# fengpeng-yue/speech-to-speech-translation

Hardware: AMD Instinct MI355X
Metric: mel-frames/sec (fwd+bwd+opt) on Fisher-shaped fbank80->mel80 (higher is better)
Workload: dtype bf16; 1 GPU; s2st_transformer base 12enc/6dec d512 nfps4 + aux ASR/ST(1x64) + CTC, recipe dropouts, max-tokens=20000 Fisher-shaped batches, update-freq 1; parallelism=dp1

## Files before the change

speech-to-speech-translation_amd/csrc/gemm_bf16.hip:

```cpp
#include "gemm_bf16_tile.h"
#include "gemm_bf16_launch.h"

namespace {

template <int BM, int BN, bool AKM, bool BKM, bool VEC>
__global__ __launch_bounds__(256) void gemm_bf16_kernel(GemmArgs g) {
  constexpr int WM = BM / 2, WN = BN / 2, TM = WM / 16, TN = WN / 16;
  typedef Stage<AKM, BM, VEC> LA;
  typedef Stage<BKM, BN, VEC> LB;
  constexpr int A_BYTES = LA::BYTES, B_BYTES = LB::BYTES, STAGE = A_BYTES + B_BYTES;
  __shared__ __attribute__((aligned(16))) unsigned char smem[2 * STAGE];

  const int tid = threadIdx.x;
  const int wave = tid >> 6, lane = tid & 63;
  const int wm = wave >> 1, wn = wave & 1;

  const int nwg = gridDim.x;
  int id = blockIdx.x;
  {
    const int x = id & 7, q = nwg >> 3, r = nwg & 7;
    id = (x < r ? x * (q + 1) : r * (q + 1) + (x - r) * q) + (id >> 3);
  }
  const int tile_m = id / g.tiles_n, tile_n = id - tile_m * g.tiles_n;
  const int m0 = tile_m * BM, n0 = tile_n * BN;
// ... 663 lines not shown
  const int z = blockIdx.y, zq = z / zdiv, zr = z - zq * zdiv;
  const float* sp = slab + ((long)z * splitk * M + m) * N + n;
  float* cp = C.p + zq * C.zo + zr * C.zi + split_off(C.sp, m) + n;
  const long sstride = (long)M * N;
  if ((N & 3) == 0 && ((uintptr_t)cp & 15) == 0) {
    float4 a = accumulate ? *reinterpret_cast<const float4*>(cp) : make_float4(0.f, 0.f, 0.f, 0.f);
    for (int sb = 0; sb < splitk; sb += 8) {
      float4 v[8];
#pragma unroll
      for (int j = 0; j < 8; ++j) v[j] = *reinterpret_cast<const float4*>(sp + (long)min(sb + j, splitk - 1) * sstride);
#pragma unroll
      for (int j = 0; j < 8; ++j)
        if (sb + j < splitk) { a.x += v[j].x; a.y += v[j].y; a.z += v[j].z; a.w += v[j].w; }
    }
    *reinterpret_cast<float4*>(cp) = a;
  } else {
    for (int r = 0; r < 4 && n + r < N; ++r) {
      float a = accumulate ? cp[r] : 0.f;
      for (int s = 0; s < splitk; ++s) a += sp[s * sstride + r];
      cp[r] = a;
    }
  }
}

template <int BM, int BN, bool VEC>
int launch_staged(const GemmArgs& g, dim3 grid, hipStream_t st) {
  return with_layouts(g, [&](auto a, auto b) {
    constexpr bool AKM = decltype(a)::value, BKM = decltype(b)::value;
    return launch_configured<GEMM_STAGED, BM, BN, AKM, BKM, VEC>(gemm_bf16_kernel<BM, BN, AKM, BKM, VEC>, 0, grid, 256, st, g);
  });
}

constexpr bool kExperimental =
#ifdef S2ST_EXPERIMENTAL
    true;
#else
    false;
#endif
static_assert(GEMM_BK == BK, "the plan prices the kernels' K-step");

enum SwitchScope { SW_MEMBER, SW_GROUP, SW_SINGLE };
GemmSwitches gemm_switches(SwitchScope scope) {
  static const int dma = s2st_env_int("S2ST_GEMM_DMA", 1), target = s2st_env_int("S2ST_SPLITK_TARGET", 128),
                   wgs = s2st_env_int("S2ST_GEMM_PERSIST_WGS", 0);
  GemmSwitches sw;
  sw.dma = dma;
  sw.splitk_target = target;
  sw.persist_wgs = wgs;
  sw.persist = s2st_env_int("S2ST_GEMM_PERSIST", sw.persist);
  if (!kExperimental && sw.persist > 1) sw.persist = 1;
  if (scope == SW_MEMBER) return sw;
  sw.w4 = s2st_env_int("S2ST_GEMM_W4", sw.w4);
  sw.fast_epi = s2st_env_int("S2ST_GEMM_FAST_EPI", 1) != 0;
  sw.streamk = kExperimental ? s2st_env_int("S2ST_GEMM_STREAMK", 1) : 0;
  if (sw.streamk > 0) sw.streamk_min_steps = s2st_env_int("S2ST_STREAMK_MIN_STEPS", sw.streamk_min_steps);
  if (scope == SW_GROUP) {
    sw.group_tile = s2st_env_int("S2ST_GROUP_TILE", 0);
    sw.group_oneshot = s2st_env_int("S2ST_GROUP_ONESHOT", 1) != 0;
    return sw;
  }
  sw.p4 = s2st_env_int("S2ST_GEMM_P4", sw.p4);
  if (const char* force = s2st_env_str("S2ST_GEMM_TILE")) {
    sw.tile_set = true;
    if (sscanf(force, "%dx%d", &sw.tile_bm, &sw.tile_bn) != 2) sw.tile_bm = sw.tile_bn = 64;
  }
  return sw;
}

GemmChip gemm_chip(const GemmSwitches& sw, int ncu = 0, int slots160 = 0) {
  return GemmChip{ncu > 0 ? ncu : num_cus(sw), slots160 > 0 ? slots160 : s2st_gemm_bf16_w4_slots160(), kExperimental};
}

GemmGroup group_of(const GemmArgs* list, const GemmPlan& p) {
  GemmGroup grp{};
  grp.n = p.n;
  grp.total = p.total;
  for (int i = 0; i < p.n; ++i) {
    GemmArgs& g = grp.g[i] = list[i];
    if (g.zdiv <= 0) g.zdiv = 1;
    g.avec = g.bvec = p.vec;
    g.cvec = p.cvec_of[i];
    g.splitk = 1;
    g.slab = nullptr;
    g.kchunk = ((g.K + BK - 1) / BK) * BK;
    g.tiles_n = (g.N + p.bn - 1) / p.bn;
    grp.tile0[i + 1] = p.tile0[i + 1];
  }
  return grp;
}

}

void s2st_gemm_streamk_bind(hipStream_t st, float* scratch, long floats) {
  if (floats < S2ST_STREAMK_SCRATCH_FLOATS) scratch = nullptr;
  for (int i = 0; i < g_sk_n; ++i)
    if (g_sk[i].st == st) { g_sk[i].p = scratch; return; }
  if (g_sk_n < 4) g_sk[g_sk_n++] = SkScratch{st, scratch};
}
void s2st_gemm_streamk_unbind_all() { g_sk_n = 0; }

bool s2st_gemm_group_ok(const GemmArgs& g) {
  return group_member_ok(g, gemm_switches(SW_MEMBER));
}

int s2st_gemm_bf16_group(const GemmArgs* list, int n, hipStream_t st) {
  if (n <= 0) return 0;
  const GemmSwitches sw = gemm_switches(SW_GROUP);
  const GemmPlan p = plan_group(list, n, sw, gemm_chip(sw), sk_scratch(st) != nullptr);
  if (p.error) return p.error;
  GemmGroup grp = group_of(list, p);
  grp.xcd_global = 1;
  int rc = S2ST_ERR_ARG;
  switch (p.form) {
    case GEMM_GROUP_RING: rc = launch_group_ring(grp, st); break;
    case GEMM_GROUP_W4: rc = s2st_gemm_bf16_w4_group(grp, st); break;
#ifdef S2ST_EXPERIMENTAL
    case GEMM_GROUP_PERSISTENT: rc = launch_persistent<128, 128>(grp, p.sk, p.grid_x, st); break;
    case GEMM_GROUP_PERSISTENT_256: rc = launch_persistent<256, 128>(grp, p.sk, p.grid_x, st); break;
#endif
    default: break;
  }
  return rc == 0 && hipGetLastError() == hipSuccess ? 0 : S2ST_ERR_LAUNCH;
}

int s2st_gemm_bf16_preload(hipStream_t st) {
  dim3 grid(1, 1, 1);
  int rc = 0;
  for (int lay = 0; lay < 4; ++lay) {
    const GemmArgs g = empty_problem(lay);
    rc |= launch_staged<128, 128, true>(g, grid, st);
    rc |= launch_staged<128, 64, true>(g, grid, st);
    rc |= launch_staged<64, 64, true>(g, grid, st);
    rc |= launch_staged<64, 64, false>(g, grid, st);
    rc |= launch_ring<128, 128>(g, grid, st);
    rc |= launch_ring<128, 64>(g, grid, st);
    if (g.A.kmajor) rc |= launch_ring<160, 64>(g, grid, st);
    rc |= launch_ring<64, 64>(g, grid, st);
    GemmGroup grp{};
    grp.n = 1;
    grp.g[0] = g;
#ifdef S2ST_EXPERIMENTAL
    rc |= launch_persistent<128, 128>(grp, false, 1, st);
    rc |= launch_persistent<128, 64>(grp, false, 1, st);
    rc |= launch_persistent<256, 128>(grp, false, 1, st);
    rc |= launch_ring<256, 128>(g, grid, st);
#endif
    rc |= launch_group_ring(grp, st);
  }
  rc |= s2st_gemm_bf16_w4_preload(st);
  rc |= s2st_gemm_bf16_p4_preload(st);
  return rc || hipGetLastError() != hipSuccess ? -1 : 0;
}

int s2st_gemm_bf16(GemmArgs g, hipStream_t st, int* tile_out) {
  const GemmSwitches sw = gemm_switches(SW_SINGLE);
  const GemmPlan p = plan_single(g, sw, gemm_chip(sw), sk_scratch(st) != nullptr);
  if (p.error) return p.error;
  g.avec = g.bvec = p.vec;
  g.cvec = p.cvec;
  g.splitk = p.splitk;
  g.kchunk = p.kchunk;
  g.tiles_n = p.tiles_n;
  g.slab = p.use_slab ? g.ws : nullptr;
  if (tile_out) *tile_out = p.bm * 1000 + p.bn;
  const dim3 grid(p.grid_x, p.grid_y, 1);
  const bool wide = p.bn == 128;
  int rc = S2ST_ERR_ARG;
  switch (p.form) {
    case GEMM_STAGED:
      rc = !p.vec ? launch_staged<64, 64, false>(g, grid, st) : p.bm == 64 ? launch_staged<64, 64, true>(g, grid, st)
           : wide ? launch_staged<128, 128, true>(g, grid, st) : launch_staged<128, 64, true>(g, grid, st);
      break;
    case GEMM_RING:
      rc = p.bm == 160 ? launch_ring<160, 64>(g, grid, st) : p.bm == 64 ? launch_ring<64, 64>(g, grid, st)
           : wide ? launch_ring<128, 128>(g, grid, st) : launch_ring<128, 64>(g, grid, st);
      break;
    case GEMM_W4: rc = s2st_gemm_bf16_w4(g, p.bm, p.bn, grid, st); break;
    case GEMM_P4: rc = s2st_gemm_bf16_p4(g, grid, st); break;
#ifdef S2ST_EXPERIMENTAL
    case GEMM_RING_256x128: rc = launch_ring<256, 128>(g, grid, st); break;
    case GEMM_PERSISTENT:
      rc = wide ? launch_persistent<128, 128>(group_of(&g, p), p.sk, p.grid_x, st)
                : launch_persistent<128, 64>(group_of(&g, p), p.sk, p.grid_x, st);
      break;
#endif
    default: break;
  }
  if (rc) return rc;
  if (p.use_slab) {
    const long nthr = (long)g.M * ((g.N + 3) / 4);
    const double by = 4.0 * g.M * g.N * g.batch * (g.splitk + 1 + (g.ep.accumulate ? 1 : 0));
    s2st_launch("splitk_reduce_kernel", by, 0.0, splitk_reduce_kernel, dim3((unsigned)((nthr + 255) / 256), g.batch),
                dim3(256), 0, st, (const float*)g.slab, g.C, g.M, g.N, g.splitk, g.zdiv, g.ep.accumulate);
  }
  return hipGetLastError() == hipSuccess ? 0 : -1;
}

int s2st_gemm_bf16_plan(const GemmArgs* list, int n, int ncu, int slots160, bool sk_bound, s2st_gemm_plan_info* out) {
  const GemmSwitches sw = gemm_switches(n ? SW_GROUP : SW_SINGLE);
  const GemmChip chip = gemm_chip(sw, ncu, slots160);
  GemmPlan p;
  if (list[0].A.dtype != S2ST_BF16 || list[0].B.dtype != S2ST_BF16 || list[0].precise) p.error = S2ST_ERR_ARG;
  else if (n == 0) p = plan_single(list[0], sw, chip, sk_bound);
  else {
    for (int i = 0; i < n && !p.error; ++i)
      if (!group_member_ok(list[i], sw)) p.error = S2ST_ERR_SHAPE;
    if (!p.error) p = plan_group(list, n, sw, chip, sk_bound);
  }
  *out = s2st_gemm_plan_info{p.error};
  if (p.error) return 0;
  *out = s2st_gemm_plan_info{0, (int)p.form, p.bm, p.bn, p.splitk, p.kchunk, p.tiles_n, p.use_slab, p.vec, p.cvec, p.grid_x, p.grid_y,
                             p.sk, p.n, p.total};
// ... 218 lines not shown
```

speech-to-speech-translation_amd/csrc/gemm_bf16_plan.h:

```cpp
#pragma once
#include <stdint.h>
#include <stdio.h>
#include "s2st_hip.h"

typedef s2st_gemm_operand GemmOperand;
typedef s2st_gemm_args GemmArgs;

constexpr int GEMM_BK = 64;
#define S2ST_GROUP_MAX 8
#define S2ST_STREAMK_MAX_WGS 512
#define S2ST_STREAMK_SCRATCH_FLOATS (1024 + (long)S2ST_STREAMK_MAX_WGS * 128 * 128)

struct GemmSwitches {
  int dma = 1;
  bool tile_set = false;
  int tile_bm = 64, tile_bn = 64;
  int w4 = -1;
  int p4 = -1;
  int persist = 1;
  int persist_wgs = 0;
  int streamk = 1;
  int streamk_min_steps = 8;
  bool fast_epi = true;
  int splitk_target = 128;
  int group_tile = 0;
  bool group_oneshot = true;
};

struct GemmChip { int ncu; int slots160; bool experimental; };

enum GemmForm {
  GEMM_STAGED, GEMM_RING, GEMM_W4, GEMM_P4, GEMM_PERSISTENT, GEMM_RING_256x128,
  GEMM_GROUP_RING, GEMM_GROUP_W4, GEMM_GROUP_PERSISTENT, GEMM_GROUP_PERSISTENT_256
};

struct GemmPlan {
  int error = 0;
  GemmForm form = GEMM_STAGED;
  int bm = 0, bn = 0, splitk = 1, kchunk = 0, tiles_n = 0, vec = 0, cvec = 0, grid_x = 0, grid_y = 1;
  bool use_slab = false;
  bool akm = false, bkm = false;
  bool sk = false;
  int n = 0, total = 0, tile0[S2ST_GROUP_MAX + 1] = {0}, cvec_of[S2ST_GROUP_MAX] = {0};
};

constexpr int ring_ns(int bm) { return bm == 256 ? 3 : 4; }
constexpr int ring_nw(int bm) { return bm == 64 ? 4 : 8; }
constexpr bool ring_il(int bm) { return bm != 256; }
constexpr int W4_NS = 2;

inline void gemm_tag(char* buf, size_t cap, GemmForm f, int bm, int bn, bool akm, bool bkm, bool last) {
  const char *a = akm ? "true" : "false", *b = bkm ? "true" : "false", *l = last ? "true" : "false";
  switch (f) {
    case GEMM_STAGED: snprintf(buf, cap, "gemm_bf16_kernel<%d, %d, %s, %s, %s>", bm, bn, a, b, l); break;
    case GEMM_RING: case GEMM_RING_256x128: case GEMM_GROUP_RING:
      snprintf(buf, cap, "gemm_bf16_dma%s_kernel<%d, %d, %s, %s, %d, %d, %s>", f == GEMM_GROUP_RING ? "_group" : "", bm, bn, a, b,
               ring_ns(bm), ring_nw(bm), ring_il(bm) ? "true" : "false");
      break;
    case GEMM_W4: case GEMM_GROUP_W4:
      snprintf(buf, cap, "gemm_bf16_w4%s_kernel<%d, %d, %s, %s, %d>", f == GEMM_GROUP_W4 ? "_group" : "", bm, bn, a, b, W4_NS);
      break;
    case GEMM_P4: snprintf(buf, cap, "gemm_bf16_p4_kernel<256, 256>"); break;
    default:
      snprintf(buf, cap, "gemm_bf16_dma_persistent_kernel<%d, %d, %s, %s, %d, %d, %s>", bm, bn, a, b, ring_ns(bm), ring_nw(bm), l);
  }
}

inline long gemm_tiles(const GemmArgs& g, int bm, int bn) { return (long)((g.M + bm - 1) / bm) * ((g.N + bn - 1) / bn) * g.batch; }

inline bool vec_ok(const GemmOperand& o) {
  return ((uintptr_t)o.p % 16 == 0) && (o.sp.ld % 8 == 0) && (o.sp.bs % 8 == 0) && (o.zo % 8 == 0) && (o.zi % 8 == 0);
}

inline bool dma_layout_ok(const GemmArgs& g) { return (g.A.kmajor || g.A.sp.per <= 0) && (g.B.kmajor || g.B.sp.per <= 0); }

inline bool prep_flags(const GemmArgs& g, int* cvec) {
  *cvec = ((!g.C.p || (uintptr_t)g.C.p % 16 == 0) && (!g.C.h || (uintptr_t)g.C.h % 8 == 0) &&
           g.C.sp.ld % 4 == 0 && g.C.sp.bs % 4 == 0 && g.C.zo % 4 == 0 && g.C.zi % 4 == 0 &&
           (!g.ep.resid || (uintptr_t)g.ep.resid % 16 == 0) && (!g.ep.bias || ((uintptr_t)g.ep.bias % 16 == 0 && g.ep.bias_zo % 4 == 0)))
              ? 1 : 0;
  return vec_ok(g.A) && vec_ok(g.B);
}

inline int mark_fast_epilogue(const GemmArgs& g, int cvec, bool unsplit, const GemmSwitches& sw) {
  cvec &= 1;
  if (!sw.fast_epi) return cvec;
  const bool drop = g.ep.drop_p > 0.f, res = g.ep.resid != nullptr, accu = g.ep.accumulate != 0;
  const bool combo = !accu || (!drop && !res && !g.C.h);
  const bool h16 = !g.C.h || ((uintptr_t)g.C.h % 16 == 0 && g.C.sp.ld % 8 == 0 && g.C.sp.bs % 8 == 0 && g.C.zo % 8 == 0 &&
                              g.C.zi % 8 == 0 && g.N % 8 == 0);
  if (cvec && g.N >= 4 && g.N % 4 == 0 && g.M >= 1 && unsplit && !g.ep.mask_y && !g.ep.colsum && !g.ep.colsum_part &&
      (g.ep.act != 2 || (!drop && !accu)) && combo && h16 && (g.C.p || g.C.h) && (!accu || g.C.p))
    cvec |= 2;
  if (cvec && g.ep.mask_y && g.C.h && !g.C.p && h16 && g.N >= 8 && g.M >= 1 && unsplit && !g.ep.bias &&
      g.ep.act == 0 && !drop && !res && !accu && (uintptr_t)g.ep.mask_y % 16 == 0)
    cvec |= 8;
  return cvec;
}

inline bool tile160_ok(const GemmArgs& g) { return g.A.kmajor && g.A.sp.per <= 0 && g.batch == 1; }

inline int w4_pick(const GemmArgs& g, const GemmSwitches& sw, const GemmChip& chip, int* bm) {
  *bm = 128;
  if (sw.w4 == 0 || g.M < 128) return 0;
  const long t128 = gemm_tiles(g, 128, 128), t64 = gemm_tiles(g, 128, 64);
  if (sw.w4 < 0 && t128 < chip.ncu) return 0;
  const long s128 = 2L * chip.ncu, s64 = 3L * chip.ncu;
  const double e128 = (double)t128 / (double)(((t128 + s128 - 1) / s128) * s128);
  const double e64 = (double)t64 / (double)(((t64 + s64 - 1) / s64) * s64);
  if (tile160_ok(g) && g.N > 64) {
    const long t160 = gemm_tiles(g, 160, 128);
    const long s160 = (long)chip.slots160 * chip.ncu;
    if (t160 <= s160 && t128 > s128 && t64 > s64) { *bm = 160; return 128; }
  }
  if (g.N > 64 && g.K >= 1024 && t128 >= 4 * s128) return 128;
  return (g.N > 64 && e128 >= e64) ? 128 : 64;
}

inline bool p4_can(const GemmArgs& g) {
  return g.A.kmajor && g.B.kmajor && g.batch == 1 && g.A.sp.per <= 0 && g.B.sp.per <= 0 && !g.ep.mask_y &&
         !g.ep.colsum && !g.ep.colsum_part;
}
inline bool p4_pick(const GemmArgs& g, const GemmSwitches& sw, const GemmChip& chip) {
  if (sw.p4 >= 1) return true;
  if (g.M < 512 || g.N < 512 || g.K < 8 * GEMM_BK) return false;
  const long ncu = chip.ncu;
  const long rounds = (gemm_tiles(g, 256, 256) + ncu - 1) / ncu;
  const double t_p4 = (double)rounds * (2.0 * ((g.K + GEMM_BK - 1) / GEMM_BK) + 7.0);
  const double t_ring = 2.0 * g.M * (double)g.N * g.K / 650e6;
  return t_p4 < 0.80 * t_ring;
}

inline bool streamk_pays(long total, long steps, const GemmSwitches& sw, const GemmChip& chip) {
  const int G = chip.ncu & ~7;
// ... 160 lines not shown
```

speech-to-speech-translation_amd/csrc/gemm_bf16_tile.h:

```cpp
#pragma once
#include <cstdio>
#include <cstdlib>

#include "s2st_ops.h"
#include "s2st_prof.h"

namespace {

typedef unsigned short bf16_t;
constexpr int BK = 64;

template <int ROWS>
__device__ __forceinline__ int kperm(int kr) {
  if (ROWS >= 128) return (kr & 3) | (((kr >> 3) & 1) << 2);
  return ((kr >> 1) & 1) | (((kr >> 3) & 1) << 1);
}

__device__ __forceinline__ uint4 mask_tail(uint4 v, int nvalid) {
  unsigned w[4] = {v.x, v.y, v.z, v.w};
#pragma unroll
  for (int i = 0; i < 4; ++i) {
    int e = nvalid - 2 * i;
    w[i] = e >= 2 ? w[i] : (e == 1 ? (w[i] & 0xffffu) : 0u);
  }
// ... 74 lines not shown
      if (KM) {
        const int row = f >> 3, ch = f & 7;
        o = row * 128 + ((ch ^ (row & 7)) << 4);
      } else {
        const int kr = f / RC, ch = f % RC;
        o = kr * PITCH + (((((ch >> 1) ^ kperm<ROWS>(kr)) << 1) | (ch & 1)) << 4);
      }
      *reinterpret_cast<uint4*>(img + o) = r[i];
    }
  }

  struct Raw { bf16x8 v; s16x4 lo, hi; };
  __device__ static __forceinline__ Raw raw(const unsigned char* img, int rt, int s, int lane) {
    Raw r;
    if (KM) {
      r.v = frag(img, rt, s, lane);
    } else {
      const int g = lane >> 4, q = (lane >> 2) & 3, p = lane & 3;
      const int kr = 32 * s + 8 * g + q;
      const unsigned char* a = img + kr * PITCH + ((((rt >> 4) ^ kperm<ROWS>(kr))) << 5) + 8 * p;
      r.lo = lds_read_tr16_raw(a);
      r.hi = lds_read_tr16_raw(a + 4 * PITCH);
    }
    return r;
  }
  __device__ static __forceinline__ bf16x8 done(Raw& r) {
    if (KM) return r.v;
    lds_raw_fence(r.lo);
    lds_raw_fence(r.hi);
    bf16x8 fr;
    fr[0] = r.lo[0]; fr[1] = r.lo[1]; fr[2] = r.lo[2]; fr[3] = r.lo[3];
    fr[4] = r.hi[0]; fr[5] = r.hi[1]; fr[6] = r.hi[2]; fr[7] = r.hi[3];
    return fr;
  }

  __device__ static __forceinline__ bf16x8 frag(const unsigned char* img, int rt, int s, int lane) {
    if (KM) {
      const int row = rt + (lane & 15), ch = 4 * s + (lane >> 4);
      return *reinterpret_cast<const bf16x8*>(img + row * 128 + ((ch ^ (row & 7)) << 4));
    } else {
      const int g = lane >> 4, q = (lane >> 2) & 3, p = lane & 3;
      const int kr = 32 * s + 8 * g + q;
      const unsigned char* a = img + kr * PITCH + ((((rt >> 4) ^ kperm<ROWS>(kr))) << 5) + 8 * p;
      s16x4 lo = lds_read_tr16(a);
      s16x4 hi = lds_read_tr16(a + 4 * PITCH);
      bf16x8 fr;
      fr[0] = lo[0]; fr[1] = lo[1]; fr[2] = lo[2]; fr[3] = lo[3];
      fr[4] = hi[0]; fr[5] = hi[1]; fr[6] = hi[2]; fr[7] = hi[3];
      return fr;
    }
  }
};

template <int BM, int BN, int WGN, bool DROP, bool RESID, bool ACC, bool HASC, bool HASH, bool H16, bool GELU = false>
__device__ __forceinline__ void gemm_epilogue_fast(const GemmArgs& g, f32x4 (&acc)[BM / 32][BN / (16 * WGN)], int m0, int n0,
                                                   int wm, int wn, int lane, int zb, int zq, int zr,
                                                   const float4 (*pre)[BN / (16 * WGN)]) {
  constexpr int WM = BM / 2, WN = BN / WGN, TM = WM / 16, TN = WN / 16;
  const long czoff = zq * g.C.zo + zr * g.C.zi;
  float* cbase = g.C.p + czoff;
  bf16_t* hbase = g.C.h + czoff;
  const float* rbase = g.ep.resid + czoff;
  const int M = g.M, N = g.N;
  const float alpha = g.ep.alpha, lo = g.ep.act == 1 ? 0.f : -__builtin_inff();
  const float drop_p = g.ep.drop_p, inv_keep = DROP ? 1.f / (1.f - drop_p) : 1.f;
  const uint64_t seed = g.ep.seed;
  int ncol[TN];
  bool nok[TN];
  float4 b4[TN];
#pragma unroll
  for (int j = 0; j < TN; ++j) {
    const int n = n0 + wn * WN + j * 16 + (lane >> 4) * 4;
    nok[j] = n < N;
    ncol[j] = nok[j] ? n : N - 4;
    b4[j] = make_float4(0.f, 0.f, 0.f, 0.f);
  }
  if (g.ep.bias) {
    const float* bias = g.ep.bias + zq * g.ep.bias_zo;
#pragma unroll
    for (int j = 0; j < TN; ++j) b4[j] = *reinterpret_cast<const float4*>(bias + ncol[j]);
  }
  long roff[TM];
  int mrow[TM];
  bool mok[TM];
#pragma unroll
  for (int i = 0; i < TM; ++i) {
    const int m = m0 + wm * WM + i * 16 + (lane & 15);
    mok[i] = m < M;
    mrow[i] = mok[i] ? m : M - 1;
    roff[i] = split_off(g.C.sp, mrow[i]);
  }
  float4 r4[RESID ? TM : 1][RESID ? TN : 1], c4[ACC ? TM : 1][ACC ? TN : 1];
  if (RESID) {
#pragma unroll
    for (int i = 0; i < TM; ++i)
#pragma unroll
      for (int j = 0; j < TN; ++j)
        r4[RESID ? i : 0][RESID ? j : 0] = pre ? pre[i][j] : *reinterpret_cast<const float4*>(rbase + roff[i] + ncol[j]);
  }
  if (ACC) {
#pragma unroll
    for (int i = 0; i < TM; ++i)
#pragma unroll
      for (int j = 0; j < TN; ++j)
        c4[ACC ? i : 0][ACC ? j : 0] = pre ? pre[i][j] : *reinterpret_cast<const float4*>(cbase + roff[i] + ncol[j]);
  }
  uint2 hp[(HASH && H16) ? TM : 1][(HASH && H16) ? TN : 1];
#pragma unroll
  for (int i = 0; i < TM; ++i) {
#pragma unroll
    for (int j = 0; j < TN; ++j) {
      float v[4] = {fmaxf(alpha * acc[i][j][0] + b4[j].x, lo), fmaxf(alpha * acc[i][j][1] + b4[j].y, lo),
                    fmaxf(alpha * acc[i][j][2] + b4[j].z, lo), fmaxf(alpha * acc[i][j][3] + b4[j].w, lo)};
      if (GELU) {
#pragma unroll
        for (int r = 0; r < 4; ++r) v[r] = gelu_erf_fast(v[r]);
      }
      if (DROP) {
        const uint64_t e0 = ((uint64_t)zb * M + mrow[i]) * (uint64_t)N + ncol[j];
#pragma unroll
        for (int r = 0; r < 4; ++r) v[r] *= drop_scale(seed, e0 + r, drop_p, inv_keep);
      }
      if (RESID) {
        const float4 t = r4[RESID ? i : 0][RESID ? j : 0];
        v[0] += t.x; v[1] += t.y; v[2] += t.z; v[3] += t.w;
      }
      if (ACC) {
        const float4 t = c4[ACC ? i : 0][ACC ? j : 0];
        v[0] += t.x; v[1] += t.y; v[2] += t.z; v[3] += t.w;
      }
      if (mok[i] && nok[j]) {
        if (HASC) *reinterpret_cast<float4*>(cbase + roff[i] + ncol[j]) = make_float4(v[0], v[1], v[2], v[3]);
        if (HASH && !H16) *reinterpret_cast<uint2*>(hbase + roff[i] + ncol[j]) = pack_bf16x4(v[0], v[1], v[2], v[3]);
      }
      if (HASH && H16) hp[(HASH && H16) ? i : 0][(HASH && H16) ? j : 0] = pack_bf16x4(v[0], v[1], v[2], v[3]);
    }
  }
  if (HASH && H16) {
    const bool odd = (lane >> 4) & 1;
#pragma unroll
    for (int i = 0; i + 1 < TM; i += 2) {
#pragma unroll
      for (int j = 0; j < TN; ++j) {
        unsigned ax = hp[i][j].x, ay = hp[i][j].y, bx = hp[i + 1][j].x, by = hp[i + 1][j].y;
        lane16_swap(ax, bx);
        lane16_swap(ay, by);
        const int n = n0 + wn * WN + j * 16 + ((lane >> 4) & 2) * 4;
        const bool ok = (odd ? mok[i + 1] : mok[i]) && n < N;
        const long ro = odd ? roff[i + 1] : roff[i];
        if (ok) *reinterpret_cast<uint4*>(hbase + ro + n) = make_uint4(ax, ay, bx, by);
      }
    }
    if constexpr (TM % 2 == 1) {
#pragma unroll
      for (int j = 0; j < TN; ++j)
        if (mok[TM - 1] && nok[j]) *reinterpret_cast<uint2*>(hbase + roff[TM - 1] + ncol[j]) = hp[TM - 1][j];
    }
  }
}

template <int BM, int BN, int WGN>
__device__ __forceinline__ void gemm_epilogue_fast_masky(const GemmArgs& g, f32x4 (&acc)[BM / 32][BN / (16 * WGN)], int m0, int n0,
                                                         int wm, int wn, int lane, int zq, int zr) {
  constexpr int WM = BM / 2, WN = BN / WGN, TM = WM / 16, TN = WN / 16;
  const long czoff = zq * g.C.zo + zr * g.C.zi;
  bf16_t* hbase = g.C.h + czoff;
  const bf16_t* ybase = g.ep.mask_y + czoff;
  const int M = g.M, N = g.N;
  const float alpha = g.ep.alpha * g.ep.mask_scale;
  int ncol[TN];
  bool nok[TN];
#pragma unroll
  for (int j = 0; j < TN; ++j) {
    const int n = n0 + wn * WN + j * 16 + (lane >> 4) * 4;
    nok[j] = n < N;
    ncol[j] = nok[j] ? n : N - 4;
  }
  long roff[TM];
  bool mok[TM];
  uint2 y4[TM][TN];
#pragma unroll
  for (int i = 0; i < TM; ++i) {
    const int m = m0 + wm * WM + i * 16 + (lane & 15);
    mok[i] = m < M;
    roff[i] = split_off(g.C.sp, mok[i] ? m : M - 1);
#pragma unroll
    for (int j = 0; j < TN; ++j) y4[i][j] = *reinterpret_cast<const uint2*>(ybase + roff[i] + ncol[j]);
  }
  float cs[TN][4];
#pragma unroll
  for (int j = 0; j < TN; ++j) cs[j][0] = cs[j][1] = cs[j][2] = cs[j][3] = 0.f;
  uint2 hp[TM][TN];
#pragma unroll
  for (int i = 0; i < TM; ++i) {
#pragma unroll
    for (int j = 0; j < TN; ++j) {
      const unsigned yw[4] = {y4[i][j].x & 0x7fffu, (y4[i][j].x >> 16) & 0x7fffu, y4[i][j].y & 0x7fffu, (y4[i][j].y >> 16) & 0x7fffu};
      float v[4];
#pragma unroll
      for (int r = 0; r < 4; ++r) {
        v[r] = yw[r] != 0 ? alpha * acc[i][j][r] : 0.f;
        if (mok[i] && nok[j]) cs[j][r] += v[r];
      }
      hp[i][j] = pack_bf16x4(v[0], v[1], v[2], v[3]);
    }
  }
  const bool odd = (lane >> 4) & 1;
#pragma unroll
  for (int i = 0; i + 1 < TM; i += 2) {
#pragma unroll
    for (int j = 0; j < TN; ++j) {
      unsigned ax = hp[i][j].x, ay = hp[i][j].y, bx = hp[i + 1][j].x, by = hp[i + 1][j].y;
      lane16_swap(ax, bx);
      lane16_swap(ay, by);
      const int n = n0 + wn * WN + j * 16 + ((lane >> 4) & 2) * 4;
      const bool ok = (odd ? mok[i + 1] : mok[i]) && n < N;
      const long ro = odd ? roff[i + 1] : roff[i];
      if (ok) *reinterpret_cast<uint4*>(hbase + ro + n) = make_uint4(ax, ay, bx, by);
    }
  }
  if constexpr (TM % 2 == 1) {
#pragma unroll
    for (int j = 0; j < TN; ++j)
      if (mok[TM - 1] && nok[j]) *reinterpret_cast<uint2*>(hbase + roff[TM - 1] + ncol[j]) = hp[TM - 1][j];
  }
  if (g.ep.colsum || g.ep.colsum_part) {
    float* prow = g.ep.colsum_part ? g.ep.colsum_part + ((long)(m0 / BM) * 2 + wm) * N : nullptr;
#pragma unroll
    for (int j = 0; j < TN; ++j) {
      float t[4];
#pragma unroll
      for (int r = 0; r < 4; ++r) t[r] = row16_sum(cs[j][r]);
      if ((lane & 15) == 0 && nok[j]) {
        if (prow) *reinterpret_cast<float4*>(prow + ncol[j]) = make_float4(t[0], t[1], t[2], t[3]);
        else {
#pragma unroll
          for (int r = 0; r < 4; ++r) atomicAdd(g.ep.colsum + ncol[j] + r, t[r]);
        }
      }
    }
  }
}

template <int BM, int BN, int WGN, bool DROP, bool RESID, bool ACC, bool GELU = false>
__device__ __forceinline__ void gemm_epilogue_fast_out(const GemmArgs& g, f32x4 (&acc)[BM / 32][BN / (16 * WGN)], int m0, int n0,
                                                       int wm, int wn, int lane, int zb, int zq, int zr,
                                                       const float4 (*pre)[BN / (16 * WGN)]) {
  constexpr bool PAIRS = BM / 32 >= 2;
  if constexpr (ACC) {
    gemm_epilogue_fast<BM, BN, WGN, DROP, RESID, ACC, true, false, false>(g, acc, m0, n0, wm, wn, lane, zb, zq, zr, pre);
  } else {
    if (g.C.p && g.C.h) gemm_epilogue_fast<BM, BN, WGN, DROP, RESID, ACC, true, true, PAIRS, GELU>(g, acc, m0, n0, wm, wn, lane, zb, zq, zr, pre);
    else if (g.C.p) gemm_epilogue_fast<BM, BN, WGN, DROP, RESID, ACC, true, false, false, GELU>(g, acc, m0, n0, wm, wn, lane, zb, zq, zr, pre);
    else gemm_epilogue_fast<BM, BN, WGN, DROP, RESID, ACC, false, true, PAIRS, GELU>(g, acc, m0, n0, wm, wn, lane, zb, zq, zr, pre);
  }
}

template <int BM, int BN, int WGN, bool FAST = false>
__device__ __forceinline__ void gemm_epilogue(const GemmArgs& g, f32x4 (&acc)[BM / 32][BN / (16 * WGN)], int m0,
                                              int n0, int wm, int wn, int lane, int zb, int ks, int zq, int zr,
                                              const float4 (*pre)[BN / (16 * WGN)] = nullptr) {
  constexpr int WM = BM / 2, WN = BN / WGN, TM = WM / 16, TN = WN / 16;
  const long czoff = zq * g.C.zo + zr * g.C.zi;
  float* cbase = g.C.p ? g.C.p + czoff : nullptr;
  bf16_t* hbase = g.C.h ? g.C.h + czoff : nullptr;
  const float* rbase = g.ep.resid ? g.ep.resid + czoff : nullptr;
  const float inv_keep = g.ep.drop_p > 0.f ? 1.f / (1.f - g.ep.drop_p) : 1.f;
  const bool lead = (ks == 0);
  const bool cvec = g.cvec != 0;
  if constexpr (FAST) {
  if (g.cvec & 8) {
    gemm_epilogue_fast_masky<BM, BN, WGN>(g, acc, m0, n0, wm, wn, lane, zq, zr);
    return;
  }
  if (g.cvec & 2) {
    const bool drop = g.ep.drop_p > 0.f, res = g.ep.resid != nullptr, accu = g.ep.accumulate != 0;
    if (g.ep.act == 2) {
      if (res) gemm_epilogue_fast_out<BM, BN, WGN, false, true, false, true>(g, acc, m0, n0, wm, wn, lane, zb, zq, zr, pre);
      else gemm_epilogue_fast_out<BM, BN, WGN, false, false, false, true>(g, acc, m0, n0, wm, wn, lane, zb, zq, zr, pre);
    } else
    if (!drop && !res && !accu) gemm_epilogue_fast_out<BM, BN, WGN, false, false, false>(g, acc, m0, n0, wm, wn, lane, zb, zq, zr, pre);
    else if (!drop && res && !accu) gemm_epilogue_fast_out<BM, BN, WGN, false, true, false>(g, acc, m0, n0, wm, wn, lane, zb, zq, zr, pre);
    else if (!drop && !res && accu) gemm_epilogue_fast_out<BM, BN, WGN, false, false, true>(g, acc, m0, n0, wm, wn, lane, zb, zq, zr, pre);
    else if (drop && !res && !accu) gemm_epilogue_fast_out<BM, BN, WGN, true, false, false>(g, acc, m0, n0, wm, wn, lane, zb, zq, zr, pre);
    else gemm_epilogue_fast_out<BM, BN, WGN, true, true, false>(g, acc, m0, n0, wm, wn, lane, zb, zq, zr, pre);
    return;
  }
  }
  if (g.slab) {
    float* sb = g.slab + (long)blockIdx.y * g.M * g.N;
    const bool v4 = (g.N & 3) == 0;
#pragma unroll
    for (int i = 0; i < TM; ++i) {
      const int m = m0 + wm * WM + i * 16 + (lane & 15);
      if (m >= g.M) continue;
#pragma unroll
      for (int j = 0; j < TN; ++j) {
        const int n = n0 + wn * WN + j * 16 + (lane >> 4) * 4;
        if (n >= g.N) continue;
        float* dst = sb + (long)m * g.N + n;
        if (v4) {
          *reinterpret_cast<float4*>(dst) = make_float4(g.ep.alpha * acc[i][j][0], g.ep.alpha * acc[i][j][1],
                                                        g.ep.alpha * acc[i][j][2], g.ep.alpha * acc[i][j][3]);
        } else {
#pragma unroll
          for (int r = 0; r < 4; ++r) if (n + r < g.N) dst[r] = g.ep.alpha * acc[i][j][r];
        }
      }
    }
    return;
  }
  const bf16_t* ybase = g.ep.mask_y ? g.ep.mask_y + czoff : nullptr;
  float cs[TN][4];
#pragma unroll
  for (int j = 0; j < TN; ++j) cs[j][0] = cs[j][1] = cs[j][2] = cs[j][3] = 0.f;
#pragma unroll
  for (int i = 0; i < TM; ++i) {
    const int m = m0 + wm * WM + i * 16 + (lane & 15);
    if (m >= g.M) continue;
    const long roff = split_off(g.C.sp, m);
#pragma unroll
    for (int j = 0; j < TN; ++j) {
// ... 182 lines not shown
```

speech-to-speech-translation_amd/runtime/binding.py:

```python
from __future__ import annotations

import collections
import ctypes as C
import os
from typing import Optional

import torch

_HERE = os.path.dirname(os.path.abspath(__file__))
DEFAULT_LIB = os.path.join(os.path.dirname(_HERE), "csrc", "libs2st_hip.so")

_lib: Optional[C.CDLL] = None
_lib_is_emulator = False


class Split(C.Structure):
    _fields_ = [("ld", C.c_int64), ("bs", C.c_int64), ("per", C.c_int32), ("_pad", C.c_int32)]


class GemmOperand(C.Structure):
    _fields_ = [("p", C.c_void_p), ("kmajor", C.c_int32), ("dtype", C.c_int32), ("sp", Split),
                ("zo", C.c_int64), ("zi", C.c_int64)]


# ... 28 lines not shown
            f"{path} not found: build it with `python -c 'import __graft_entry__ as g; g.build()'`"
            " (hipcc --offload-arch=gfx950). There is no CPU fallback.")
    _lib = C.CDLL(path)
    _lib_is_emulator = emulator
    for name, (ret, alist) in header_prototypes().items():
        fn = getattr(_lib, name, None)
        if fn is not None:
            fn.restype, fn.argtypes = ret, [t for t, _ in alist]
    return _lib


def lib() -> C.CDLL:
    if _lib is None:
        load_library()
    return _lib


def is_emulator() -> bool:
    return _lib_is_emulator


def check(rc: int, what: str):
    if rc != 0:
        raise S2STHipError(f"{what} failed with code {rc}")


def ptr(t: Optional[torch.Tensor]) -> Optional[int]:
    if t is None:
        return None
    return t.data_ptr()


def stream_ptr() -> Optional[int]:
    if _lib_is_emulator or not torch.cuda.is_available():
        return None
    return torch.cuda.current_stream().cuda_stream


def require_device(t: torch.Tensor):
    if not _lib_is_emulator and not t.is_cuda:
        raise S2STHipError("s2st HIP ops need device (cuda/HIP) tensors; there is no CPU path")


def make_split(ld: int, per: int = 0, bs: int = 0) -> Split:
    return Split(ld, bs, per, 0)


def gemm(A: torch.Tensor, B: torch.Tensor, Cout: torch.Tensor, M: int, N: int, K: int, *,
         a_kmajor=True, a_ld=None, a_per=0, a_bs=0, a_zo=0, a_zi=0,
         b_kmajor=True, b_ld=None, b_per=0, b_bs=0, b_zo=0, b_zi=0,
         c_ld=None, c_per=0, c_bs=0, c_zo=0, c_zi=0,
         batch=1, zdiv=1, alpha=1.0, bias=None, act=0, drop_p=0.0, seed=0, resid=None,
         accumulate=False, precise=False, a_off=0, b_off=0, c_off=0, c_bf16=None, ws=None,
         mask_y=None, mask_scale=1.0, colsum=None, return_tile=False):
    require_device(A)
    if A.dtype != B.dtype:
        raise S2STHipError("gemm operands must have the same dtype")
    if A.dtype == torch.bfloat16:
        return _gemm_bf16(A, B, Cout, M, N, K, locals())
    g = GemmArgs()
    g.A = GemmOperand(A.data_ptr() + 4 * a_off, 1 if a_kmajor else 0, 0,
                      make_split(a_ld if a_ld is not None else (K if a_kmajor else M), a_per, a_bs),
                      a_zo, a_zi)
    g.B = GemmOperand(B.data_ptr() + 4 * b_off, 1 if b_kmajor else 0, 0,
                      make_split(b_ld if b_ld is not None else (K if b_kmajor else N), b_per, b_bs),
                      b_zo, b_zi)
    g.C = GemmOut(Cout.data_ptr() + 4 * c_off, make_split(c_ld if c_ld is not None else N, c_per, c_bs),
                  c_zo, c_zi, None)
    g.ep = GemmEpilogue(alpha, act, ptr(bias), drop_p, 1 if accumulate else 0, seed, ptr(resid), None, 1.0, None)
    g.M, g.N, g.K, g.batch, g.zdiv, g.precise = M, N, K, batch, zdiv, 1 if precise else 0
    check(lib().s2st_gemm_f32(C.byref(g), C.c_void_p(stream_ptr())), "s2st_gemm_f32")


def _gemm_bf16(A, B, Cout, M, N, K, kw):
    g = GemmArgs()
    a_ld = kw["a_ld"] if kw["a_ld"] is not None else (K if kw["a_kmajor"] else M)
    b_ld = kw["b_ld"] if kw["b_ld"] is not None else (K if kw["b_kmajor"] else N)
    g.A = GemmOperand(A.data_ptr() + 2 * kw["a_off"], 1 if kw["a_kmajor"] else 0, 1,
                      make_split(a_ld, kw["a_per"], kw["a_bs"]), kw["a_zo"], kw["a_zi"])
    g.B = GemmOperand(B.data_ptr() + 2 * kw["b_off"], 1 if kw["b_kmajor"] else 0, 1,
                      make_split(b_ld, kw["b_per"], kw["b_bs"]), kw["b_zo"], kw["b_zi"])
    h = kw["c_bf16"]
    g.C = GemmOut(Cout.data_ptr() + 4 * kw["c_off"] if Cout is not None else None,
                  make_split(kw["c_ld"] if kw["c_ld"] is not None else N, kw["c_per"], kw["c_bs"]),
                  kw["c_zo"], kw["c_zi"], h.data_ptr() + 2 * kw["c_off"] if h is not None else None)
    g.ep = GemmEpilogue(kw["alpha"], kw["act"], ptr(kw["bias"]), kw["drop_p"], 1 if kw["accumulate"] else 0,
                        kw["seed"], ptr(kw["resid"]), ptr(kw.get("mask_y")), kw.get("mask_scale", 1.0),
                        ptr(kw.get("colsum")))
    g.M, g.N, g.K, g.batch, g.zdiv, g.precise = M, N, K, kw["batch"], kw["zdiv"], 0
    if kw["ws"] is not None:
        g.ws, g.ws_floats = kw["ws"].data_ptr(), kw["ws"].numel()
    if kw.get("return_tile"):
        t = C.c_int32(0)
        check(lib().s2st_gemm_tile_f32(C.byref(g), C.byref(t), C.c_void_p(stream_ptr())), "s2st_gemm_tile_f32")
        return (t.value // 1000, t.value % 1000)
    check(lib().s2st_gemm_f32(C.byref(g), C.c_void_p(stream_ptr())), "s2st_gemm_f32")


def gemm_args_bf16(A, B, Cout, M, N, K, *, a_kmajor=True, b_kmajor=True, a_ld=None, b_ld=None, c_ld=None, bias=None,
                   act=0, resid=None, accumulate=False, c_bf16=None, alpha=1.0) -> GemmArgs:
    g = GemmArgs()
    g.A = GemmOperand(A.data_ptr(), 1 if a_kmajor else 0, 1, make_split(a_ld or (K if a_kmajor else M)), 0, 0)
    g.B = GemmOperand(B.data_ptr(), 1 if b_kmajor else 0, 1, make_split(b_ld or (K if b_kmajor else N)), 0, 0)
    g.C = GemmOut(ptr(Cout), make_split(c_ld or N), 0, 0, ptr(c_bf16))
    g.ep = GemmEpilogue(alpha, act, ptr(bias), 0.0, 1 if accumulate else 0, 0, ptr(resid), None, 1.0, None)
    g.M, g.N, g.K, g.batch, g.zdiv, g.precise = M, N, K, 1, 1, 0
    return g


def gemm_group(problems):
    arr = (GemmArgs * len(problems))(*problems)
    check(lib().s2st_gemm_group_f32(arr, len(problems), C.c_void_p(stream_ptr())), "s2st_gemm_group_f32")


class GemmPlanInfo(C.Structure):
    _fields_ = [(k, C.c_int32) for k in ("error", "form", "bm", "bn", "splitk", "kchunk", "tiles_n", "use_slab", "vec", "cvec",
                                         "grid_x", "grid_y", "sk", "n", "total")] + \
               [("cvec_of", C.c_int32 * 8), ("tag", C.c_char * 104)]


GEMM_FORMS = ("STAGED", "RING", "W4", "P4", "PERSISTENT", "RING_256x128", "GROUP_RING", "GROUP_W4", "GROUP_PERSISTENT",
              "GROUP_PERSISTENT_256")
GemmPlan = collections.namedtuple("GemmPlan", "error form tag bm bn splitk kchunk tiles_n use_slab vec cvec grid sk n total cvec_of")


def gemm_plan(args, ncu=0, slots160=0, sk_bound=False, _info=GemmPlanInfo()) -> GemmPlan:
    p = _info
    if isinstance(args, GemmArgs):
        rc = lib().s2st_gemm_plan_f32(C.byref(args), ncu, slots160, 1 if sk_bound else 0, C.byref(p))
    else:
        arr = (GemmArgs * len(args))(*args)
        rc = lib().s2st_gemm_group_plan_f32(arr, len(args), ncu, slots160, 1 if sk_bound else 0, C.byref(p))
    check(rc, "s2st_gemm_plan_f32")
    if p.error:
        return GemmPlan(p.error, None, None, 0, 0, 0, 0, 0, False, False, 0, (0, 0), False, 0, 0, ())
    return GemmPlan(0, GEMM_FORMS[p.form], p.tag.decode(), p.bm, p.bn, p.splitk, p.kchunk, p.tiles_n, bool(p.use_slab), bool(p.vec),
                    p.cvec, (p.grid_x, p.grid_y), bool(p.sk), p.n, p.total, tuple(p.cvec_of[:p.n]))


class AttnArgs(C.Structure):
    _fields_ = [("q", C.c_void_p), ("k", C.c_void_p), ("v", C.c_void_p), ("ldq", C.c_int64), ("ldk", C.c_int64),
# ... 172 lines not shown
```

Measured before the change: 1.500 million mel-frames/s.

## Shuffle GEMM epilogue fragments into row-contiguous 16-byte bf16 stores and loads

Adds a row-oriented epilogue mode, on by default and switchable via S2ST_EPI_ROWS. It uses cross-lane shuffles to regroup MFMA accumulator fragments so that each lane writes, and for the masked-y path reads, 16-byte contiguous bf16 row segments instead of scattered 8-byte column chunks. This mode is applied to ring, w4 and persistent forms but not to the staged or p4 kernels. It aims to cut the number of global memory transactions in the epilogue, at the cost of extra shuffle instructions and register pressure. The Python binding also gains a colsum_part argument.

```diff
diff --git a/speech-to-speech-translation_amd/csrc/gemm_bf16.hip b/speech-to-speech-translation_amd/csrc/gemm_bf16.hip
--- a/speech-to-speech-translation_amd/csrc/gemm_bf16.hip
+++ b/speech-to-speech-translation_amd/csrc/gemm_bf16.hip
@@ -739,6 +739,7 @@
   if (scope == SW_MEMBER) return sw;
   sw.w4 = s2st_env_int("S2ST_GEMM_W4", sw.w4);
   sw.fast_epi = s2st_env_int("S2ST_GEMM_FAST_EPI", 1) != 0;
+  sw.epi_rows = s2st_env_int("S2ST_EPI_ROWS", 1) != 0;
   sw.streamk = kExperimental ? s2st_env_int("S2ST_GEMM_STREAMK", 1) : 0;
   if (sw.streamk > 0) sw.streamk_min_steps = s2st_env_int("S2ST_STREAMK_MIN_STEPS", sw.streamk_min_steps);
   if (scope == SW_GROUP) {
@@ -796,6 +797,7 @@
   const GemmPlan p = plan_group(list, n, sw, gemm_chip(sw), sk_scratch(st) != nullptr);
   if (p.error) return p.error;
   GemmGroup grp = group_of(list, p);
+  for (int i = 0; i < p.n; ++i) grp.g[i].cvec = launch_cvec(grp.g[i].cvec, p.form, sw);
   grp.xcd_global = 1;
   int rc = S2ST_ERR_ARG;
   switch (p.form) {
@@ -844,7 +846,7 @@
   const GemmPlan p = plan_single(g, sw, gemm_chip(sw), sk_scratch(st) != nullptr);
   if (p.error) return p.error;
   g.avec = g.bvec = p.vec;
-  g.cvec = p.cvec;
+  g.cvec = launch_cvec(p.cvec, p.form, sw);
   g.splitk = p.splitk;
   g.kchunk = p.kchunk;
   g.tiles_n = p.tiles_n;
diff --git a/speech-to-speech-translation_amd/csrc/gemm_bf16_plan.h b/speech-to-speech-translation_amd/csrc/gemm_bf16_plan.h
--- a/speech-to-speech-translation_amd/csrc/gemm_bf16_plan.h
+++ b/speech-to-speech-translation_amd/csrc/gemm_bf16_plan.h
@@ -22,6 +22,7 @@
   int streamk = 1;
   int streamk_min_steps = 8;
   bool fast_epi = true;
+  bool epi_rows = true;
   int splitk_target = 128;
   int group_tile = 0;
   bool group_oneshot = true;
@@ -80,6 +81,11 @@
            (!g.ep.resid || (uintptr_t)g.ep.resid % 16 == 0) && (!g.ep.bias || ((uintptr_t)g.ep.bias % 16 == 0 && g.ep.bias_zo % 4 == 0)))
               ? 1 : 0;
   return vec_ok(g.A) && vec_ok(g.B);
+}
+
+constexpr int GEMM_CVEC_ROWS = 16;
+inline int launch_cvec(int cvec, GemmForm form, const GemmSwitches& sw) {
+  return (sw.epi_rows && (cvec & 10) && form != GEMM_P4 && form != GEMM_STAGED) ? cvec | GEMM_CVEC_ROWS : cvec;
 }
 
 inline int mark_fast_epilogue(const GemmArgs& g, int cvec, bool unsplit, const GemmSwitches& sw) {
diff --git a/speech-to-speech-translation_amd/csrc/gemm_bf16_tile.h b/speech-to-speech-translation_amd/csrc/gemm_bf16_tile.h
--- a/speech-to-speech-translation_amd/csrc/gemm_bf16_tile.h
+++ b/speech-to-speech-translation_amd/csrc/gemm_bf16_tile.h
@@ -150,6 +150,112 @@
   }
 };
 
+__device__ __forceinline__ int rows_src(int lane) { return (lane & 3) * 16 + (lane >> 2); }
+template <int TM, int TN>
+__device__ __forceinline__ constexpr bool rows_fit() { return TM * TN < 16; }
+
+template <int TN>
+__device__ __forceinline__ void store_bf16_rows_block(const GemmArgs& g, bf16_t* hbase, const uint2 (&hp)[TN], int mrow0,
+                                                      int nbase, int lane) {
+  static_assert(TN % 2 == 0, "column blocks pair up");
+  const int r = lane >> 2, c = lane & 3, sa = 32 * (c & 1) + r, sb = sa + 16, m = mrow0 + r;
+  const bool hi = c >> 1;
+  const long ro = split_off(g.C.sp, m < g.M ? m : g.M - 1);
+#pragma unroll
+  for (int jp = 0; jp < TN / 2; ++jp) {
+    const uint2 a0 = hp[2 * jp], a1 = hp[2 * jp + 1];
+    const unsigned x0 = __shfl(a0.x, sa), y0 = __shfl(a0.y, sa), z0 = __shfl(a0.x, sb), w0 = __shfl(a0.y, sb);
+    const unsigned x1 = __shfl(a1.x, sa), y1 = __shfl(a1.y, sa), z1 = __shfl(a1.x, sb), w1 = __shfl(a1.y, sb);
+    const int n = nbase + jp * 32 + c * 8;
+    if (m < g.M && n < g.N)
+      *reinterpret_cast<uint4*>(hbase + ro + n) = hi ? make_uint4(x1, y1, z1, w1) : make_uint4(x0, y0, z0, w0);
+  }
+}
+
+template <int TM, int TN>
+__device__ __forceinline__ void store_bf16_rows(const GemmArgs& g, bf16_t* hbase, const uint2 (&hp)[TM][TN], int mbase,
+                                                int nbase, int lane) {
+  static_assert(TN == 1 || TN % 2 == 0, "column blocks pair up");
+  const int M = g.M, N = g.N;
+  if constexpr (TN > 1) {
+#pragma unroll
+    for (int i = 0; i < TM; ++i) store_bf16_rows_block<TN>(g, hbase, hp[i], mbase + i * 16, nbase, lane);
+  } else {
+    const int r = lane >> 1, sa = 32 * (lane & 1) + (r & 15), sb = sa + 16;
+    const bool hi = r >> 4;
+#pragma unroll
+    for (int i = 0; i + 1 < TM; i += 2) {
+      const int m = mbase + i * 16 + r;
+      const long ro = split_off(g.C.sp, m < M ? m : M - 1);
+      const uint2 a0 = hp[i][0], a1 = hp[i + 1][0];
+      const unsigned x0 = __shfl(a0.x, sa), y0 = __shfl(a0.y, sa), z0 = __shfl(a0.x, sb), w0 = __shfl(a0.y, sb);
+      const unsigned x1 = __shfl(a1.x, sa), y1 = __shfl(a1.y, sa), z1 = __shfl(a1.x, sb), w1 = __shfl(a1.y, sb);
+      const int n = nbase + (lane & 1) * 8;
+      if (m < M && n < N)
+        *reinterpret_cast<uint4*>(hbase + ro + n) = hi ? make_uint4(x1, y1, z1, w1) : make_uint4(x0, y0, z0, w0);
+    }
+    if constexpr (TM % 2 == 1) {
+      const int m = mbase + (TM - 1) * 16 + (lane >> 2), n = nbase + (lane & 3) * 4;
+      const unsigned x = __shfl(hp[TM - 1][0].x, rows_src(lane)), y = __shfl(hp[TM - 1][0].y, rows_src(lane));
+      if (m < M && n < N) *reinterpret_cast<uint2*>(hbase + split_off(g.C.sp, m) + n) = make_uint2(x, y);
+    }
+  }
+}
+
+template <int TN>
+__device__ __forceinline__ void load_bf16_rows_block(const GemmArgs& g, const bf16_t* ybase, uint4 (&w)[TN / 2], int mrow0,
+                                                     int nbase, int lane) {
+  static_assert(TN % 2 == 0, "column blocks pair up");
+  const int m = mrow0 + (lane >> 2);
+  const long ro = split_off(g.C.sp, m < g.M ? m : g.M - 1);
+#pragma unroll
+  for (int jp = 0; jp < TN / 2; ++jp) {
+    const int n = nbase + jp * 32 + (lane & 3) * 8;
+    w[jp] = *reinterpret_cast<const uint4*>(ybase + ro + (n < g.N ? n : g.N - 8));
+  }
+}
+template <int TN>
+__device__ __forceinline__ void take_bf16_rows_block(const uint4 (&w)[TN / 2], uint2 (&y4)[TN], int lane) {
+  const int rr = lane & 15, gq = lane >> 4;
+  const bool odd = gq & 1;
+#pragma unroll
+  for (int j = 0; j < TN; ++j) {
+    const uint4 p = w[j >> 1];
+    const int s = 4 * rr + 2 * (j & 1) + (gq >> 1);
+    const unsigned x = __shfl(p.x, s), y = __shfl(p.y, s), z = __shfl(p.z, s), ww = __shfl(p.w, s);
+    y4[j] = odd ? make_uint2(z, ww) : make_uint2(x, y);
+  }
+}
+
+template <int TM, int TN>
+__device__ __forceinline__ void load_bf16_rows(const GemmArgs& g, const bf16_t* ybase, uint2 (&y4)[TM][TN], int mbase,
+                                               int nbase, int lane) {
+  static_assert(TN == 1, "wider waves work row block by row block: load_bf16_rows_block / take_bf16_rows_block");
+  const int M = g.M, N = g.N;
+  const int rr = lane & 15, gq = lane >> 4;
+  const bool odd = gq & 1;
+  {
+    const int r = lane >> 1;
+#pragma unroll
+    for (int i = 0; i + 1 < TM; i += 2) {
+      const int m = mbase + i * 16 + r, n = nbase + (lane & 1) * 8;
+      const uint4 w = *reinterpret_cast<const uint4*>(ybase + split_off(g.C.sp, m < M ? m : M - 1) + (n < N ? n : N - 8));
+#pragma unroll
+      for (int b = 0; b < 2; ++b) {
+        const int s = 2 * (16 * b + rr) + (gq >> 1);
+        const unsigned x = __shfl(w.x, s), y = __shfl(w.y, s), z = __shfl(w.z, s), ww = __shfl(w.w, s);
+        y4[i + b][0] = odd ? make_uint2(z, ww) : make_uint2(x, y);
+      }
+    }
+    if constexpr (TM % 2 == 1) {
+      const int m = mbase + (TM - 1) * 16 + (lane >> 2), n = nbase + (lane & 3) * 4;
+      const uint2 w = *reinterpret_cast<const uint2*>(ybase + split_off(g.C.sp, m < M ? m : M - 1) + (n < N ? n : N - 4));
+      const int s = 4 * rr + gq;
+      y4[TM - 1][0] = make_uint2(__shfl(w.x, s), __shfl(w.y, s));
+    }
+  }
+}
+
 template <int BM, int BN, int WGN, bool DROP, bool RESID, bool ACC, bool HASC, bool HASH, bool H16, bool GELU = false>
 __device__ __forceinline__ void gemm_epilogue_fast(const GemmArgs& g, f32x4 (&acc)[BM / 32][BN / (16 * WGN)], int m0, int n0,
                                                    int wm, int wn, int lane, int zb, int zq, int zr,
@@ -163,12 +269,16 @@
   const float alpha = g.ep.alpha, lo = g.ep.act == 1 ? 0.f : -__builtin_inff();
   const float drop_p = g.ep.drop_p, inv_keep = DROP ? 1.f / (1.f - drop_p) : 1.f;
   const uint64_t seed = g.ep.seed;
+  constexpr bool FIRST = HASC || RESID || ACC;
+  const bool rows = rows_fit<TM, TN>() && (g.cvec & GEMM_CVEC_ROWS) != 0, moved = FIRST && rows;
+  const int lrow = moved ? lane >> 2 : lane & 15, lcg = moved ? lane & 3 : lane >> 4;
+  const int msrc = moved ? rows_src(lane) : lane;
   int ncol[TN];
   bool nok[TN];
   float4 b4[TN];
 #pragma unroll
   for (int j = 0; j < TN; ++j) {
-    const int n = n0 + wn * WN + j * 16 + (lane >> 4) * 4;
+    const int n = n0 + wn * WN + j * 16 + lcg * 4;
     nok[j] = n < N;
     ncol[j] = nok[j] ? n : N - 4;
     b4[j] = make_float4(0.f, 0.f, 0.f, 0.f);
@@ -183,33 +293,43 @@
   bool mok[TM];
 #pragma unroll
   for (int i = 0; i < TM; ++i) {
-    const int m = m0 + wm * WM + i * 16 + (lane & 15);
+    const int m = m0 + wm * WM + i * 16 + lrow;
     mok[i] = m < M;
     mrow[i] = mok[i] ? m : M - 1;
     roff[i] = split_off(g.C.sp, mrow[i]);
   }
   float4 r4[RESID ? TM : 1][RESID ? TN : 1], c4[ACC ? TM : 1][ACC ? TN : 1];
+  auto handed = [&](const float4 t) {
+    if (!moved) return t;
+    const int src = rows_src(lane);
+    return make_float4(__shfl(t.x, src), __shfl(t.y, src), __shfl(t.z, src), __shfl(t.w, src));
+  };
   if (RESID) {
 #pragma unroll
     for (int i = 0; i < TM; ++i)
 #pragma unroll
       for (int j = 0; j < TN; ++j)
-        r4[RESID ? i : 0][RESID ? j : 0] = pre ? pre[i][j] : *reinterpret_cast<const float4*>(rbase + roff[i] + ncol[j]);
+        r4[RESID ? i : 0][RESID ? j : 0] = pre ? handed(pre[i][j]) : *reinterpret_cast<const float4*>(rbase + roff[i] + ncol[j]);
   }
   if (ACC) {
 #pragma unroll
     for (int i = 0; i < TM; ++i)
 #pragma unroll
       for (int j = 0; j < TN; ++j)
-        c4[ACC ? i : 0][ACC ? j : 0] = pre ? pre[i][j] : *reinterpret_cast<const float4*>(cbase + roff[i] + ncol[j]);
+        c4[ACC ? i : 0][ACC ? j : 0] = pre ? handed(pre[i][j]) : *reinterpret_cast<const float4*>(cbase + roff[i] + ncol[j]);
   }
   uint2 hp[(HASH && H16) ? TM : 1][(HASH && H16) ? TN : 1];
 #pragma unroll
   for (int i = 0; i < TM; ++i) {
 #pragma unroll
     for (int j = 0; j < TN; ++j) {
-      float v[4] = {fmaxf(alpha * acc[i][j][0] + b4[j].x, lo), fmaxf(alpha * acc[i][j][1] + b4[j].y, lo),
-                    fmaxf(alpha * acc[i][j][2] + b4[j].z, lo), fmaxf(alpha * acc[i][j][3] + b4[j].w, lo)};
+      f32x4 a = acc[i][j];
+      if (moved) {
+#pragma unroll
+        for (int r = 0; r < 4; ++r) a[r] = __shfl(a[r], msrc);
+      }
+      float v[4] = {fmaxf(alpha * a[0] + b4[j].x, lo), fmaxf(alpha * a[1] + b4[j].y, lo),
+                    fmaxf(alpha * a[2] + b4[j].z, lo), fmaxf(alpha * a[3] + b4[j].w, lo)};
       if (GELU) {
 #pragma unroll
         for (int r = 0; r < 4; ++r) v[r] = gelu_erf_fast(v[r]);
@@ -234,7 +354,17 @@
       if (HASH && H16) hp[(HASH && H16) ? i : 0][(HASH && H16) ? j : 0] = pack_bf16x4(v[0], v[1], v[2], v[3]);
     }
   }
-  if (HASH && H16) {
+  if (HASH && H16 && rows) {
+    if (FIRST) {
+#pragma unroll
+      for (int i = 0; i < TM; ++i)
+#pragma unroll
+        for (int j = 0; j < TN; ++j)
+          if (mok[i] && nok[j]) *reinterpret_cast<uint2*>(hbase + roff[i] + ncol[j]) = hp[HASH && H16 ? i : 0][HASH && H16 ? j : 0];
+    } else {
+      if constexpr (HASH && H16) store_bf16_rows<TM, TN>(g, hbase, hp, m0 + wm * WM, n0 + wn * WN, lane);
+    }
+  } else if (HASH && H16) {
     const bool odd = (lane >> 4) & 1;
 #pragma unroll
     for (int i = 0; i + 1 < TM; i += 2) {
@@ -282,28 +412,69 @@
     const int m = m0 + wm * WM + i * 16 + (lane & 15);
     mok[i] = m < M;
     roff[i] = split_off(g.C.sp, mok[i] ? m : M - 1);
-#pragma unroll
-    for (int j = 0; j < TN; ++j) y4[i][j] = *reinterpret_cast<const uint2*>(ybase + roff[i] + ncol[j]);
-  }
+  }
+  const bool rows = rows_fit<TM, TN>() && (g.cvec & GEMM_CVEC_ROWS) != 0;
+  const bool odd = (lane >> 4) & 1;
   float cs[TN][4];
 #pragma unroll
   for (int j = 0; j < TN; ++j) cs[j][0] = cs[j][1] = cs[j][2] = cs[j][3] = 0.f;
-  uint2 hp[TM][TN];
-#pragma unroll
-  for (int i = 0; i < TM; ++i) {
+  auto block = [&](int i, const uint2 (&y)[TN], uint2 (&h)[TN]) {
 #pragma unroll
     for (int j = 0; j < TN; ++j) {
-      const unsigned yw[4] = {y4[i][j].x & 0x7fffu, (y4[i][j].x >> 16) & 0x7fffu, y4[i][j].y & 0x7fffu, (y4[i][j].y >> 16) & 0x7fffu};
+      const unsigned yw[4] = {y[j].x & 0x7fffu, (y[j].x >> 16) & 0x7fffu, y[j].y & 0x7fffu, (y[j].y >> 16) & 0x7fffu};
       float v[4];
 #pragma unroll
       for (int r = 0; r < 4; ++r) {
         v[r] = yw[r] != 0 ? alpha * acc[i][j][r] : 0.f;
         if (mok[i] && nok[j]) cs[j][r] += v[r];
       }
-      hp[i][j] = pack_bf16x4(v[0], v[1], v[2], v[3]);
-    }
-  }
-  const bool odd = (lane >> 4) & 1;
+      h[j] = pack_bf16x4(v[0], v[1], v[2], v[3]);
+    }
+  };
+  bool streamed = false;
+  if constexpr (TN > 1) {
+    if (rows) {
+      uint4 w[TM][TN / 2];
+#pragma unroll
+      for (int i = 0; i < TM; ++i) load_bf16_rows_block<TN>(g, ybase, w[i], m0 + wm * WM + i * 16, n0 + wn * WN, lane);
+#pragma unroll
+      for (int i = 0; i < TM; ++i) {
+        uint2 y[TN], h[TN];
+        take_bf16_rows_block<TN>(w[i], y, lane);
+        block(i, y, h);
+        store_bf16_rows_block<TN>(g, hbase, h, m0 + wm * WM + i * 16, n0 + wn * WN, lane);
+      }
+      streamed = true;
+    }
+  }
+  if (!streamed) {
+  if (rows) {
+    if constexpr (TN == 1) load_bf16_rows<TM, TN>(g, ybase, y4, m0 + wm * WM, n0 + wn * WN, lane);
+  } else {
+#pragma unroll
+  for (int i = 0; i + 1 < TM; i += 2) {
+    const long ro = odd ? roff[i + 1] : roff[i];
+#pragma unroll
+    for (int j = 0; j < TN; ++j) {
+      const int n = n0 + wn * WN + j * 16 + ((lane >> 4) & 2) * 4;
+      const uint4 w = *reinterpret_cast<const uint4*>(ybase + ro + (n < N ? n : N - 8));
+      unsigned ax = w.x, ay = w.y, bx = w.z, by = w.w;
+      lane16_swap(ax, bx);
+      lane16_swap(ay, by);
+      y4[i][j] = make_uint2(ax, ay);
+      y4[i + 1][j] = make_uint2(bx, by);
+    }
+  }
+  if constexpr (TM % 2 == 1) {
+#pragma unroll
+    for (int j = 0; j < TN; ++j) y4[TM - 1][j] = *reinterpret_cast<const uint2*>(ybase + roff[TM - 1] + ncol[j]);
+  }
+  }
+  uint2 hp[TM][TN];
+#pragma unroll
+  for (int i = 0; i < TM; ++i) block(i, y4[i], hp[i]);
+  if (rows) store_bf16_rows<TM, TN>(g, hbase, hp, m0 + wm * WM, n0 + wn * WN, lane);
+  else {
 #pragma unroll
   for (int i = 0; i + 1 < TM; i += 2) {
 #pragma unroll
@@ -321,6 +492,8 @@
 #pragma unroll
     for (int j = 0; j < TN; ++j)
       if (mok[TM - 1] && nok[j]) *reinterpret_cast<uint2*>(hbase + roff[TM - 1] + ncol[j]) = hp[TM - 1][j];
+  }
+  }
   }
   if (g.ep.colsum || g.ep.colsum_part) {
     float* prow = g.ep.colsum_part ? g.ep.colsum_part + ((long)(m0 / BM) * 2 + wm) * N : nullptr;
@@ -365,7 +538,7 @@
   const float* rbase = g.ep.resid ? g.ep.resid + czoff : nullptr;
   const float inv_keep = g.ep.drop_p > 0.f ? 1.f / (1.f - g.ep.drop_p) : 1.f;
   const bool lead = (ks == 0);
-  const bool cvec = g.cvec != 0;
+  const bool cvec = (g.cvec & 1) != 0;
   if constexpr (FAST) {
   if (g.cvec & 8) {
     gemm_epilogue_fast_masky<BM, BN, WGN>(g, acc, m0, n0, wm, wn, lane, zq, zr);
diff --git a/speech-to-speech-translation_amd/runtime/binding.py b/speech-to-speech-translation_amd/runtime/binding.py
--- a/speech-to-speech-translation_amd/runtime/binding.py
+++ b/speech-to-speech-translation_amd/runtime/binding.py
@@ -104,7 +104,7 @@
          c_ld=None, c_per=0, c_bs=0, c_zo=0, c_zi=0,
          batch=1, zdiv=1, alpha=1.0, bias=None, act=0, drop_p=0.0, seed=0, resid=None,
          accumulate=False, precise=False, a_off=0, b_off=0, c_off=0, c_bf16=None, ws=None,
-         mask_y=None, mask_scale=1.0, colsum=None, return_tile=False):
+         mask_y=None, mask_scale=1.0, colsum=None, colsum_part=None, return_tile=False):
     require_device(A)
     if A.dtype != B.dtype:
         raise S2STHipError("gemm operands must have the same dtype")
@@ -138,7 +138,7 @@
                   kw["c_zo"], kw["c_zi"], h.data_ptr() + 2 * kw["c_off"] if h is not None else None)
     g.ep = GemmEpilogue(kw["alpha"], kw["act"], ptr(kw["bias"]), kw["drop_p"], 1 if kw["accumulate"] else 0,
                         kw["seed"], ptr(kw["resid"]), ptr(kw.get("mask_y")), kw.get("mask_scale", 1.0),
-                        ptr(kw.get("colsum")))
+                        ptr(kw.get("colsum")), ptr(kw.get("colsum_part")))
     g.M, g.N, g.K, g.batch, g.zdiv, g.precise = M, N, K, kw["batch"], kw["zdiv"], 0
     if kw["ws"] is not None:
         g.ws, g.ws_floats = kw["ws"].data_ptr(), kw["ws"].numel()
```

Measured after the change: 1.513 million mel-frames/s, median of 6. Within noise of the previous version (+0.9%).
